# STLABTW/ST-DADK

Measured on NVIDIA B200. Metric: train_samples_per_s, higher is better.
Workload: dtype tf32

## Files before the change

st_dadk_b200/csrc/api.cu:

```cuda
#include <cstdarg>
#include <cstdio>
#include <cstring>

#include "layer.cuh"
#include "misc.cuh"
#include "sparse.cuh"
#include "predict.cuh"
#include "field.cuh"

using namespace stdadk;

static thread_local char g_err[512] = "";

static int fail(int code, const char* fmt, ...) {
    va_list ap;
    va_start(ap, fmt);
    vsnprintf(g_err, sizeof(g_err), fmt, ap);
    va_end(ap);
    return code;
}
static int check_launch(const char* what) {
    cudaError_t e = cudaGetLastError();
    if (e != cudaSuccess) return fail((int)e, "%s: %s", what, cudaGetErrorString(e));
    return 0;
// ... 16 lines not shown
    if (p.major != 10) return fail(-2, "libstdadk requires an sm_100 (B200) device, found sm_%d%d", p.major, p.minor);
    g_sm_count = p.multiProcessorCount;
    ok_dev = dev;
    return 0;
}
static int grid_for(long long work_items, int threads, int per_sm = 8) {
    long long blocks = (work_items + threads - 1) / threads;
    long long cap = (long long)(g_sm_count > 0 ? g_sm_count : 148) * per_sm;
    if (blocks > cap) blocks = cap;
    if (blocks < 1) blocks = 1;
    return (int)blocks;
}
static int pow2_cols(int n) {
    int c = 32;
    while (c < n) c <<= 1;
    return c;
}
static int tmem_cols_m64(int n_pad) { return pow2_cols((n_pad + 63) & ~63); }
template <typename K>
static int set_smem(K kernel, uint32_t bytes) {
    cudaError_t e = cudaFuncSetAttribute(kernel, cudaFuncAttributeMaxDynamicSharedMemorySize, (int)bytes);
    if (e != cudaSuccess) return fail((int)e, "cudaFuncSetAttribute(%u B smem): %s", bytes, cudaGetErrorString(e));
    return 0;
}

static BasisP to_basis(const stdadk_basis* b) {
    BasisP B{};
    if (b) {
        B.knots = reinterpret_cast<const float4*>(b->knots4);
        B.tknots = reinterpret_cast<const float2*>(b->tknots2);
        B.k_s = b->k_s;
        B.k_t = b->k_t;
        B.p_cov = b->p_cov;
        B.fn = b->basis_fn;
    }
    return B;
}
static PointsP to_points(const stdadk_points& p) {
    PointsP P{};
    P.coords = p.coords;
    P.t = p.t;
    P.xcov = p.xcov;
    P.index = reinterpret_cast<const long long*>(p.index);
    P.nx = p.grid_nx;
    P.ny = p.grid_ny;
    P.nt = p.grid_nt;
// ... 124 lines not shown
    REQUIRE(src && img && rows > 0 && cols > 0, "pack_image: bad arguments");
    REQUIRE((reinterpret_cast<uintptr_t>(img) & 127) == 0, "pack_image: image must be 128-byte aligned");
    int slabs = (int)ceil_div64(cols, SLAB_K);
    long long chunks = (long long)ceil_div64(rows, TILE_M) * slabs * (SLAB_FLOATS / 4);
    pack_image_kernel<<<grid_for(chunks, 256), 256, 0, (cudaStream_t)stream>>>(src, row_stride, col_stride, rows, cols,
                                                                                img, chunks, slabs);
    return check_launch("pack_image");
}

int stdadk_pack_images(const stdadk_pack_desc* descs, int n, void* stream) {
    if (int r = check_device()) return r;
    REQUIRE(descs && n >= 1 && n <= STDADK_MAX_PACK, "pack_images: 1..%d descriptors, got %d", STDADK_MAX_PACK, n);
    PackBatch B{};
    B.n = n;
    long long max_chunks = 0;
    for (int i = 0; i < n; ++i) {
        REQUIRE(descs[i].src && descs[i].img && descs[i].rows > 0 && descs[i].cols > 0, "pack_images: bad descriptor %d", i);
        REQUIRE((reinterpret_cast<uintptr_t>(descs[i].img) & 127) == 0, "pack_images: image %d must be 128-byte aligned", i);
        B.d[i] = descs[i];
        long long chunks = ceil_div64(descs[i].rows, TILE_M) * ceil_div64(descs[i].cols, SLAB_K) * (SLAB_FLOATS / 4);
        if (chunks > max_chunks) max_chunks = chunks;
    }
    dim3 grid(grid_for(max_chunks, 256, 2), n);
    pack_images_kernel<<<grid, 256, 0, (cudaStream_t)stream>>>(B);
    return check_launch("pack_images");
}

int stdadk_unpack_image(const float* img, int64_t rows, int64_t cols, float* dst, void* stream) {
    if (int r = check_device()) return r;
    REQUIRE(dst && img && rows > 0 && cols > 0, "unpack_image: bad arguments");
    int slabs = (int)ceil_div64(cols, SLAB_K);
    unpack_image_kernel<<<grid_for(rows * cols, 256), 256, 0, (cudaStream_t)stream>>>(img, rows, cols, dst, slabs);
    return check_launch("unpack_image");
}

static int check_layer(const stdadk_layer& l, const char* who) {
    REQUIRE(l.w_img && l.bias, "%s: weight image / bias is NULL", who);
    REQUIRE(l.n_out >= 1 && l.n_out <= MAX_N, "%s: n_out=%d outside [1,%d] (one UMMA N / LayerNorm row per thread)", who,
            l.n_out, MAX_N);
    REQUIRE(l.n_in >= 1, "%s: n_in=%d", who, l.n_in);
    REQUIRE((l.gamma == nullptr) == (l.beta == nullptr), "%s: gamma and beta must both be given or both NULL", who);
    REQUIRE(((reinterpret_cast<uintptr_t>(l.w_img) | reinterpret_cast<uintptr_t>(l.w_img_lo)) & 127) == 0,
            "%s: weight images must be 128-byte aligned", who);
    return 0;
}

constexpr uint32_t SMEM_LIMIT = 227 * 1024;
// ... 47 lines not shown
    K.dbg = g_predict_dbg;
    K.out_img = a->out_img;
    K.stats = a->stats;
    K.has_head = a->head ? 1 : 0;
    K.k_slabs = pad32(a->layer.n_in) / SLAB_K;
    K.n_pad = pad32(a->layer.n_out);
    K.thresh16 = dropout_thresh16(a->drop.p);
    K.drop_scale = a->drop.p > 0.0f ? 1.0f / (1.0f - a->drop.p) : 1.0f;
    const bool basis = a->basis != nullptr;
    int tiles = (int)ceil_div64(a->pts.n_rows, TILE_M);
    const int sms = g_sm_count > 0 ? g_sm_count : 148;
    const int cg = tiles >= 2 * sms ? 2 : 4;
    const bool half_tiles = 2 * tiles <= sms;
    if (half_tiles) tiles *= 2;
    K.tmem_cols = half_tiles ? tmem_cols_m64(K.n_pad) : pow2_cols(K.n_pad);
    const uint32_t smem = fwd_smem(K.n_pad, K.has_head ? K.head.q : 0, basis ? K.basis.k_s : 0, basis ? K.basis.k_t : 0,
                                   basis ? K.k_slabs * 8 : 0, cg);
    REQUIRE(smem <= SMEM_LIMIT, "layer_fwd: needs %u B of shared memory (> 227 KB): too many knots for the dense path",
            smem);
    K.n_tiles = tiles;
#define LAUNCH_FWD(B, TM, C)                                                                                 \
    do {                                                                                                     \
        if (int r = set_smem(layer_fwd_kernel<B, TM, C, (C == 2 ? 2 : 4)>, smem)) return r;                  \
        layer_fwd_kernel<B, TM, C, (C == 2 ? 2 : 4)><<<tiles, n_threads(C), smem, (cudaStream_t)stream>>>(K); \
    } while (0)
    if (basis) {
        if (half_tiles) LAUNCH_FWD(true, 64, 4);
        else if (cg == 2) LAUNCH_FWD(true, 128, 2);
        else LAUNCH_FWD(true, 128, 4);
    } else {
        if (half_tiles) LAUNCH_FWD(false, 64, 4);
        else if (cg == 2) LAUNCH_FWD(false, 128, 2);
        else LAUNCH_FWD(false, 128, 4);
    }
#undef LAUNCH_FWD
    return check_launch("layer_fwd");
}

extern "C" void stdadk_debug_counters(void* dev_u64x16) { g_predict_dbg = static_cast<unsigned long long*>(dev_u64x16); }

static int fill_pred_layers(const stdadk_layer* layers, int n_layers, PredLayerP* out, const char* who) {
    for (int l = 0; l < n_layers; ++l) {
        const stdadk_layer& y = layers[l];
        if (int r = check_layer(y, who)) return r;
        REQUIRE(l == 0 || y.n_in == layers[l - 1].n_out, "%s: block %d n_in=%d != previous n_out=%d", who, l, y.n_in,
                layers[l - 1].n_out);
        PredLayerP& L = out[l];
// ... 187 lines not shown
    K.d_beta = a->d_beta;
    K.d_head_w = a->d_head_w;
    K.d_head_b = a->d_head_b;
    K.has_head = a->head ? 1 : 0;
    K.k_slabs = a->x_img ? 0 : pad32(a->layer.n_in) / SLAB_K;
    K.k_slabs2 = a->head ? 0 : pad32(a->n_next) / SLAB_K;
    K.n_pad = pad32(a->layer.n_out);
    K.thresh16 = dropout_thresh16(a->drop.p);
    K.drop_scale = a->drop.p > 0.0f ? 1.0f / (1.0f - a->drop.p) : 1.0f;
    const bool basis = a->basis != nullptr && a->x_img == nullptr;
    constexpr int BCG = BWD_CG, BNS = BWD_NS;
    const uint32_t smem = bwd_smem(K.n_pad, K.has_head ? K.head.q : 0, basis ? K.basis.k_s : 0, basis ? K.basis.k_t : 0,
                                   basis ? K.k_slabs * 8 : 0);
    REQUIRE(smem <= SMEM_LIMIT, "layer_bwd: needs %u B of shared memory (> 227 KB)", smem);
    int tiles = (int)ceil_div64(a->pts.n_rows, TILE_M);
    const int sms = g_sm_count > 0 ? g_sm_count : 148;
    const bool half_tiles = a->x_img && 2 * tiles <= sms;
    if (half_tiles) tiles *= 2;
    K.tmem_cols = 2 * (half_tiles ? tmem_cols_m64(K.n_pad) : pow2_cols(K.n_pad));
    const bool ln = a->layer.gamma != nullptr, hd = a->head != nullptr;
#define LAUNCH_BWD(B, TM, LNV, HD)                                                                          \
    do {                                                                                                    \
        if (int r = set_smem(layer_bwd_kernel<B, TM, BCG, BNS, LNV, HD>, smem)) return r;                   \
        layer_bwd_kernel<B, TM, BCG, BNS, LNV, HD><<<tiles, n_threads(BCG), smem, (cudaStream_t)stream>>>(K); \
    } while (0)
    if (half_tiles) {
        if (ln && hd) LAUNCH_BWD(false, 64, true, true);
        else if (ln) LAUNCH_BWD(false, 64, true, false);
        else if (hd) LAUNCH_BWD(false, 64, false, true);
        else LAUNCH_BWD(false, 64, false, false);
    } else if (basis) {
        if (ln && hd) LAUNCH_BWD(true, 128, true, true);
        else if (ln) LAUNCH_BWD(true, 128, true, false);
        else if (hd) LAUNCH_BWD(true, 128, false, true);
        else LAUNCH_BWD(true, 128, false, false);
    } else {
        if (ln && hd) LAUNCH_BWD(false, 128, true, true);
        else if (ln) LAUNCH_BWD(false, 128, true, false);
        else if (hd) LAUNCH_BWD(false, 128, false, true);
        else LAUNCH_BWD(false, 128, false, false);
    }
#undef LAUNCH_BWD
    return check_launch("layer_bwd");
}

int stdadk_wgrad(const stdadk_wgrad_args* a, void* stream) {
    if (int r = check_device()) return r;
// ... 18 lines not shown
    K.stride_o = a->stride_o;
    K.stride_i = a->stride_i;
    K.n_in = a->n_in;
    K.n_out = a->n_out;
    K.a_slabs = pad32(a->n_in) / SLAB_K;
    K.dz_slabs = pad32(a->n_out) / SLAB_K;
    K.n_row_tiles = (int)ceil_div64(a->pts.n_rows, TILE_M);
    int n_tiles_n = (K.a_slabs + 7) / 8;
    K.nt_slabs = (K.a_slabs + n_tiles_n - 1) / n_tiles_n;
    K.tmem_cols = pow2_cols(K.nt_slabs * SLAB_K);
    int m_tiles = (K.dz_slabs + 3) / 4;
    int per = m_tiles * n_tiles_n;
    int sms = g_sm_count > 0 ? g_sm_count : 148;
    int splits = sms / per;
    if (splits < 1) splits = 1;
    if (splits > K.n_row_tiles) splits = K.n_row_tiles;
    const bool basis = a->basis != nullptr;
    uint32_t smem = wgrad_smem_bytes(basis ? K.basis.k_s : 0, basis ? K.basis.k_t : 0);
    REQUIRE(smem <= SMEM_LIMIT, "wgrad: needs %u B of shared memory (> 227 KB)", smem);
    dim3 grid(splits, m_tiles, n_tiles_n);
    constexpr int WCG = 2;
    if (basis) {
        if (int r = set_smem(wgrad_kernel<true, WCG>, smem)) return r;
        wgrad_kernel<true, WCG><<<grid, n_threads(WCG), smem, (cudaStream_t)stream>>>(K);
    } else {
        if (int r = set_smem(wgrad_kernel<false, WCG>, smem)) return r;
        wgrad_kernel<false, WCG><<<grid, n_threads(WCG), smem, (cudaStream_t)stream>>>(K);
    }
    return check_launch("wgrad");
}

static int dense_basis_check(int n_in, int n_out, int k_s, int k_t, int q_head, int training) {
    REQUIRE(n_out >= 1 && n_out <= MAX_N && k_s >= 0 && k_t >= 0 && n_in >= k_s + k_t && q_head >= 0 &&
                q_head <= STDADK_MAX_Q,
            "dense_basis_supported: bad sizes n_in=%d n_out=%d k_s=%d k_t=%d q_head=%d", n_in, n_out, k_s, k_t, q_head);
    const int n_pad = pad32(n_out), tab_chunks = pad32(n_in) / SLAB_K * 8;
    for (int cg : {4, 2}) {
        const uint32_t b = fwd_smem(n_pad, q_head, k_s, k_t, tab_chunks, cg);
        REQUIRE(b <= SMEM_LIMIT, "layer_fwd: needs %u B of shared memory (> 227 KB): too many knots for the dense path", b);
    }
    if (!training) return 0;
    const uint32_t bb = bwd_smem(n_pad, q_head, k_s, k_t, tab_chunks);
    REQUIRE(bb <= SMEM_LIMIT, "layer_bwd: needs %u B of shared memory (> 227 KB)", bb);
    const uint32_t wb = wgrad_smem_bytes(k_s, k_t);
    REQUIRE(wb <= SMEM_LIMIT, "wgrad: needs %u B of shared memory (> 227 KB)", wb);
    return 0;
}

int stdadk_dense_basis_supported(int32_t n_in, int32_t n_out, int32_t k_s, int32_t k_t, int32_t q_head, int32_t training) {
    return dense_basis_check(n_in, n_out, k_s, k_t, q_head, training) == 0 ? 1 : 0;
// ... 220 lines not shown
    K.sqnorms = a->sqnorms;
    K.step_count = a->step_count;
    K.beta1 = a->beta1;
    K.beta2 = a->beta2;
    K.eps = a->eps;
    K.ema_decay = a->ema_decay;
    K.g_zero = a->zero_grad ? const_cast<float*>(a->g) : nullptr;
    K.loss_acc = a->loss_acc;
    K.loss_sum = a->loss_sum;
    K.loss_last = a->loss_last;
    REQUIRE(((reinterpret_cast<uintptr_t>(a->p) | reinterpret_cast<uintptr_t>(a->g) | reinterpret_cast<uintptr_t>(a->m) |
              reinterpret_cast<uintptr_t>(a->v) | reinterpret_cast<uintptr_t>(a->shadow)) & 15) == 0,
            "adamw: buffers must be 16-byte aligned");
    if (a->fuse_norm) {
        REQUIRE(a->norm_ws, "adamw: fuse_norm needs norm_ws");
        K.sq_out = const_cast<float*>(a->sqnorms);
        K.norm_ws = a->norm_ws;
        K.step_rw = a->step_count;
        long long blocks = ((a->n + 3) / 4 + 255) / 256;
        if (blocks > 148) blocks = 148;
        const int sms = g_sm_count > 0 ? g_sm_count : 148;
        if (blocks > sms) blocks = sms;
        if (blocks < 1) blocks = 1;
        adamw_ema_kernel<true><<<(int)blocks, 256, 0, (cudaStream_t)stream>>>(K);
        return check_launch("adamw_ema_step (fused tail)");
    }
    step_inc_kernel<<<1, 1, 0, (cudaStream_t)stream>>>(a->step_count);
    adamw_ema_kernel<false><<<grid_for((a->n + 3) / 4, 256, 8), 256, 0, (cudaStream_t)stream>>>(K);
    return check_launch("adamw_ema_step");
}

}
```

st_dadk_b200/csrc/layer.cuh:

```cuda
#pragma once
#include "common.cuh"

namespace stdadk {

constexpr int WG_NSTAGE = 2;
constexpr int RED_STRIDE = 4 + STDADK_MAX_Q;
__host__ __device__ constexpr int n_work(int cg) { return 128 * cg; }
__host__ __device__ constexpr int n_threads(int cg) { return 128 * cg + 64; }
__device__ __forceinline__ void worker_barrier(int nw) { asm volatile("bar.sync 1, %0;" ::"r"(nw) : "memory"); }

template <int TM>
struct TileGeo {
    static_assert(TM == 128 || TM == 64, "tile height");
    static constexpr int ROWS_PER_WARP = TM / 4;
    static constexpr int WARP_COLS = TM == 128 ? 32 : 64;
    __device__ static int row(int q4, int lane) { return q4 * ROWS_PER_WARP + (TM == 128 ? lane : (lane & 15)); }
    __device__ static int chunk_off(int lane) { return TM == 128 ? 0 : (lane >> 4) * 32; }
    __device__ static int group(int cg, int lane) { return TM == 128 ? cg : 2 * cg + (lane >> 4); }
    __host__ __device__ static constexpr int groups(int cg) { return TM == 128 ? cg : 2 * cg; }
};
template <int TM>
__device__ __forceinline__ void acc_ld(uint32_t taddr, float (&v)[32]) {
    if (TM == 128) tmem_ld32(taddr, v);
    else tmem_ld16x2<32>(taddr, v);
// ... 303 lines not shown
    }
    for (; c < c_end; ++c) {
        const int f = slab * SLAB_K + 4 * c;
        const float4 v = chunk_value(chunk_kind(B, f), f);
        const uint32_t so = ((uint32_t)c ^ r7) << 4;
        st_shared_v4(rbase + so, v.x, v.y, v.z, v.w);
        if (grow) *reinterpret_cast<float4*>(grow + so) = v;
    }
}

__device__ __forceinline__ void gen_basis_slab(const BasisP& B, const float4* sk, const float2* st, int slab,
                                               float x, float y, float t, const float* xrow, uint32_t slab_saddr,
                                               uint32_t r, int c_begin = 0, int c_end = 8, float* gslab = nullptr,
                                               bool lo = false) {
#pragma unroll 1
    for (int c = c_begin; c < c_end; ++c) {
        float4 v = feature_chunk(B, sk, st, slab * SLAB_K + c * 4, x, y, t, xrow, lo);
        st_shared_v4(slab_saddr + swz_off(r, c), v.x, v.y, v.z, v.w);
        if (gslab)
            *reinterpret_cast<float4*>(reinterpret_cast<uint8_t*>(gslab) + swz_off(r, c)) = v;
    }
}

__device__ __forceinline__ void issue_slab_copies(const float* w_img, int w_slabs, int slab, int n_pad,
                                                  const float* a_tile_img, float* sA, float* sB, uint64_t* bar,
                                                  uint32_t a_bytes = SLAB_BYTES) {
    uint32_t bytes = (uint32_t)n_pad * 128u + (a_tile_img ? a_bytes : 0u);
    mbar_arrive_expect_tx(bar, bytes);
    for (int r0 = 0; r0 < n_pad; r0 += TILE_M) {
        int rows = min(TILE_M, n_pad - r0);
        const float* src = w_img + ((size_t)(r0 / TILE_M) * w_slabs + slab) * SLAB_FLOATS;
        bulk_g2s(sB + (size_t)r0 * SLAB_K, src, (uint32_t)rows * 128u, bar);
    }
    if (a_tile_img) bulk_g2s(sA, a_tile_img + (size_t)slab * SLAB_FLOATS, a_bytes, bar);
}

__device__ __forceinline__ void stage_knots_async(const BasisP& B, float4* sk, float2* st, uint64_t* bar) {
    const uint32_t ks_bytes = (uint32_t)B.k_s * 16u, kt_bytes = ((uint32_t)B.k_t >> 1) * 16u;
    mbar_arrive_expect_tx(bar, ks_bytes + kt_bytes);
    if (ks_bytes) bulk_g2s(sk, B.knots, ks_bytes, bar);
    if (kt_bytes) bulk_g2s(st, B.tknots, kt_bytes, bar);
    if (B.k_t & 1) st[B.k_t - 1] = B.tknots[B.k_t - 1];
}

__device__ __forceinline__ void issue_slab_mma(uint32_t tmem_acc, const float* sA, const float* sB, uint32_t idesc,
                                               bool first) {
    uint64_t ad = umma_desc_sw128(smem_u32(sA), 16, 1024);
    uint64_t bd = umma_desc_sw128(smem_u32(sB), 16, 1024);
#pragma unroll
    for (int k = 0; k < 4; ++k) umma_tf32(tmem_acc, ad + (uint64_t)(k * 2), bd + (uint64_t)(k * 2), idesc,
                                          (first && k == 0) ? 0u : 1u);
}

__device__ __forceinline__ bool pass_a_lo(int p) { return p == 2; }
__device__ __forceinline__ bool pass_b_lo(int p) { return p == 1; }
__device__ __forceinline__ void store_operand_chunk(float* img, float* img_lo, int tile, int slabs, int c0, uint32_t row,
                                                    const float (&v)[32]) {
// ... 376 lines not shown
    for (int i = tid; i < n_pad; i += NT) {
        bool ok = i < n_out;
        sbias[i] = ok ? P.L.bias[i] : 0.0f;
        sgam[i] = (ok && has_ln) ? P.L.gamma[i] : 1.0f;
        sbet[i] = (ok && has_ln) ? P.L.beta[i] : 0.0f;
    }
    if (P.has_head) {
        for (int i = tid; i < P.head.q * n_pad; i += NT) {
            int k = i / n_pad, c = i - k * n_pad;
            shw[i] = c < n_out ? P.head.w[(size_t)k * n_out + c] : 0.0f;
        }
        if (tid < P.head.q) shb[tid] = P.head.b[tid];
    }
    tc_fence_before();
    __syncthreads();
    tc_fence_after();
    const uint32_t tmem_base = *tmem_slot;
    FWD_T(0);

    if (warp == 4 * CG) {
        if (lane == 0) {
            const size_t a_off = (size_t)itile * P.k_slabs * SLAB_FLOATS + (size_t)irow0 * SLAB_K;
            const int n_virt = P.k_slabs * P.passes;
            for (int v = 0; v < n_virt; ++v) {
                const int s = v / P.passes, p = v - s * P.passes;
                int stage = v % NSTAGE, it = v / NSTAGE;
                if (it > 0) FWD_WAIT(7, mbar_wait(&empty[stage], (it - 1) & 1));
                const float* w_src = pass_b_lo(p) ? P.L.w_img_lo : P.L.w_img;
                const float* a_tile = BASIS ? nullptr : (pass_a_lo(p) ? P.a_img_lo : P.a_img) + a_off;
                issue_slab_copies(w_src, P.k_slabs, s, n_pad, a_tile, sA + (size_t)stage * SLAB_FLOATS,
                                  sB + stage * b_stage_floats, &full[stage], TM * 128u);
            }
        }
        __syncwarp();
    } else if (warp == 4 * CG + 1) {
        if (lane == 0) {
            const uint32_t idesc = umma_idesc_tf32((uint32_t)n_pad, 0, 0, TM);
            const int n_virt = P.k_slabs * P.passes;
            for (int s = 0; s < n_virt; ++s) {
                int stage = s % NSTAGE, it = s / NSTAGE;
                FWD_WAIT(6, mbar_wait(&full[stage], it & 1));
                tc_fence_after();
                issue_slab_mma(tmem_base, sA + (size_t)stage * SLAB_FLOATS, sB + stage * b_stage_floats, idesc,
                               s == 0);
                umma_commit(&empty[stage]);
            }
            umma_commit(accf);
        }
        __syncwarp();
    } else {
        const int q4 = warp & 3, cg = warp >> 2;
        const int row = G::row(q4, lane), grp = G::group(cg, lane);
        const long long lrow = (long long)tile * TM + row;
        const bool rvalid = tile_valid && lrow < P.pts.n_rows;
        const long long grow = P.pts.row_begin + lrow;
        if (BASIS) {
            float x = 0.f, y = 0.f, t = 0.f;
            const float* xrow = nullptr;
            if (rvalid) {
                load_point(P.pts, grow, x, y, t);
                if (P.basis.p_cov > 0 && P.pts.xcov) xrow = P.pts.xcov + sample_of(P.pts, grow) * P.basis.p_cov;
            }
            auto gen_all = [&](auto fn_tag) {
                constexpr int FN = decltype(fn_tag)::value;
                int stage = 0, it = 0;
                for (int s = 0; s < P.k_slabs; ++s) {
                    float* gslab = (P.feat_img && tile_valid)
                                       ? P.feat_img + ((size_t)itile * P.k_slabs + s) * SLAB_FLOATS + (size_t)irow0 * SLAB_K
                                       : nullptr;
                    for (int p = 0; p < P.passes; ++p) {
                        if (it > 0) {
                            if (tid == 0) FWD_WAIT(5, mbar_wait(&empty[stage], (it - 1) & 1));
                            else mbar_wait(&empty[stage], (it - 1) & 1);
// ... 100 lines not shown
    if (BASIS) build_chunk_tables(P.basis, ctab, P.k_slabs * 8, tid, NT);
    for (int i = tid; i < n_pad; i += NT) {
        bool ok = i < n_out;
        sbias[i] = ok ? P.L.bias[i] : 0.0f;
        sgam[i] = (ok && has_ln) ? P.L.gamma[i] : 1.0f;
        sbet[i] = (ok && has_ln) ? P.L.beta[i] : 0.0f;
    }
    for (int i = tid; i < (3 + q) * n_pad + STDADK_MAX_Q; i += NT) cs_bias[i] = 0.0f;
    if (HEAD) {
        for (int i = tid; i < q * n_pad; i += NT) {
            int k = i / n_pad, c = i - k * n_pad;
            shw[i] = c < n_out ? P.head.w[(size_t)k * n_out + c] : 0.0f;
        }
    }
    tc_fence_before();
    __syncthreads();
    tc_fence_after();
    const uint32_t tmem_base = *tmem_slot;

    if (warp == 4 * CG) {
        if (lane == 0) {
            const size_t a_off = (size_t)itile * P.k_slabs * SLAB_FLOATS + (size_t)irow0 * SLAB_K;
            const size_t dzn_off = (size_t)itile * P.k_slabs2 * SLAB_FLOATS + (size_t)irow0 * SLAB_K;
            for (int v = 0; v < total_slabs; ++v) {
                int stage = v % NSTAGE, it = v / NSTAGE;
                if (it > 0) mbar_wait(&empty[stage], (it - 1) & 1);
                float* a_dst = sA + (size_t)stage * SLAB_FLOATS;
                float* b_dst = sB + stage * b_stage_floats;
                if (v < virt1) {
                    const int s = v / P.passes, p = v - s * P.passes;
                    const float* a_tile = BASIS ? nullptr : (pass_a_lo(p) ? P.a_img_lo : P.a_img) + a_off;
                    issue_slab_copies(pass_b_lo(p) ? P.L.w_img_lo : P.L.w_img, P.k_slabs, s, n_pad, a_tile, a_dst, b_dst,
                                      &full[stage], TM * 128u);
                } else {
                    const int s = (v - virt1) / P.passes, p = (v - virt1) - s * P.passes;
                    issue_slab_copies(pass_b_lo(p) ? P.wt_next_img_lo : P.wt_next_img, P.k_slabs2, s, n_pad,
                                      (pass_a_lo(p) ? P.dz_next_img_lo : P.dz_next_img) + dzn_off, a_dst, b_dst, &full[stage],
                                      TM * 128u);
                }
            }
        }
        __syncwarp();
    } else if (warp == 4 * CG + 1) {
        if (lane == 0) {
            const uint32_t idesc = umma_idesc_tf32((uint32_t)n_pad, 0, 0, TM);
            for (int s = 0; s < total_slabs; ++s) {
                int stage = s % NSTAGE, it = s / NSTAGE;
                mbar_wait(&full[stage], it & 1);
                tc_fence_after();
                bool second = s >= virt1;
                issue_slab_mma(tmem_base + (second ? acc1_off : 0u), sA + (size_t)stage * SLAB_FLOATS,
                               sB + stage * b_stage_floats, idesc, s == 0 || s == virt1);
                umma_commit(&empty[stage]);
            }
            umma_commit(accf);
        }
        __syncwarp();
    } else {
        const int q4 = warp & 3, cg = warp >> 2;
        const int row = G::row(q4, lane), irow = irow0 + row, grp = G::group(cg, lane), coff = G::chunk_off(lane);
        const int c_begin = grp * (8 / NG), c_end = (grp + 1) * (8 / NG);
        const long long lrow = (long long)tile * TM + row;
        const bool rvalid = lrow < P.pts.n_rows;
// ... 8 lines not shown
            auto gen_all = [&](auto fn_tag) {
                constexpr int FN = decltype(fn_tag)::value;
                for (int v = 0; v < total_slabs; ++v) {
                    int stage = v % NSTAGE, it = v / NSTAGE;
                    if (it > 0) mbar_wait(&empty[stage], (it - 1) & 1);
                    if (v < virt1) {
                        const int s = v / P.passes, p = v - s * P.passes;
                        const uint32_t sa = smem_u32(sA + (size_t)stage * SLAB_FLOATS);
                        if (pass_a_lo(p))
                            gen_basis_slab_soa<FN, true, 2>(P.basis, ctab, s, x, y, t, xrow, sa, (uint32_t)row, c_begin,
                                                            c_end, nullptr);
                        else
                            gen_basis_slab_soa<FN, false, 2>(P.basis, ctab, s, x, y, t, xrow, sa, (uint32_t)row, c_begin,
                                                             c_end, nullptr);
                        fence_proxy_async_smem();
                    }
                    mbar_arrive_warp(&full[stage]);
                }
            };
            if (P.basis.fn == STDADK_WENDLAND) gen_all(std::integral_constant<int, STDADK_WENDLAND>{});
            else if (P.basis.fn == STDADK_TRIANGULAR) gen_all(std::integral_constant<int, STDADK_TRIANGULAR>{});
            else gen_all(std::integral_constant<int, STDADK_GAUSSIAN>{});
        }
        mbar_wait(accf, 0);
        tc_fence_after();
        const uint32_t trow = tmem_base + ((uint32_t)(q4 * 32) << 16);
        float* myred = red + ((size_t)grp * TM + row) * RED_STRIDE;
        const float* arow = (P.addend && rvalid) ? P.addend + (size_t)lrow * n_out : nullptr;
        float mean = 0.0f, rstd = 1.0f;
        if (has_ln && rvalid) {
            mean = P.stats[2 * lrow];
            rstd = P.stats[2 * lrow + 1];
        }
        float dyh[STDADK_MAX_Q];
#pragma unroll
        for (int k = 0; k < STDADK_MAX_Q; ++k)
            dyh[k] = (HEAD && rvalid && k < q) ? P.head.dyhat[lrow * q + k] : 0.0f;
        const bool drop = P.L.drop_p > 0.0f;
        const unsigned int drop_step = drop ? dropout_step(P.L) : 0u;
        const float inv_n = 1.0f / (float)n_out;
        uint32_t actbits[MAXCH];
        float Sa = 0.0f, Sb = 0.0f;
        float z[32], g[32], tmp[32];

        int ch = 0;
        for (int wc = G::WARP_COLS * cg; wc < n_pad; wc += WSTEP, ++ch) {
// ... 181 lines not shown
        if (u < units_a)
            va[j] = __ldg(reinterpret_cast<const float4*>(a_tile + (size_t)(nslab0 + (u >> 9)) * SLAB_FLOATS + hoff) + (u & 511));
    }
#pragma unroll
    for (int j = 0; j < BD; ++j) {
        const int u = tid + j * NW;
        if (u < units_d) {
            const int c = u >> 9, w = u & 511;
            const uint32_t r = (uint32_t)(w >> 3), lc = (uint32_t)(w & 7) ^ (r & 7u);
            st_shared_v4(sa + c * WG_CHUNK_BYTES + swz32_off(r, lc), vd[j].x, vd[j].y, vd[j].z, vd[j].w);
        }
    }
#pragma unroll
    for (int j = 0; j < BA; ++j) {
        const int u = tid + j * NW;
        if (u < units_a) {
            const int c = u >> 9, w = u & 511;
            const uint32_t r = (uint32_t)(w >> 3), lc = (uint32_t)(w & 7) ^ (r & 7u);
            st_shared_v4(sb + c * WG_CHUNK_BYTES + swz32_off(r, lc), va[j].x, va[j].y, va[j].z, va[j].w);
        }
    }
}

template <bool BASIS, int CG>
__global__ void __launch_bounds__(n_threads(CG), 1) wgrad_kernel(const __grid_constant__ WgradK P) {
    constexpr int NW = n_work(CG), NT = n_threads(CG);
    extern __shared__ uint8_t smem_raw[];
    uint8_t* smem = align_smem(smem_raw);
    uint8_t* stage_base = smem;
    uint64_t* full = reinterpret_cast<uint64_t*>(smem + WG_NSTAGE * WG_STAGE_BYTES);
    uint64_t* empty = full + WG_NSTAGE;
    uint64_t* accf = full + 2 * WG_NSTAGE;
    uint64_t* kbar = accf + 1;
    uint32_t* tmem_slot = reinterpret_cast<uint32_t*>(smem + WG_NSTAGE * WG_STAGE_BYTES + 64);
    float4* sk = reinterpret_cast<float4*>(smem + WG_NSTAGE * WG_STAGE_BYTES + 96);
    float2* st = reinterpret_cast<float2*>(reinterpret_cast<uint8_t*>(sk) + (size_t)(BASIS ? P.basis.k_s : 0) * 16);

    const int tid = threadIdx.x, warp = tid >> 5, lane = tid & 31;
    const int split = blockIdx.x, n_split = gridDim.x, mi = blockIdx.y, ni = blockIdx.z;
    const int m_chunks = min(4, P.dz_slabs - mi * 4);
    const int n_chunks = min(P.nt_slabs, P.a_slabs - ni * P.nt_slabs);
    const int n_mma = n_chunks * SLAB_K;
    int my_tiles = 0;
    for (int rt = split; rt < P.n_row_tiles; rt += n_split) ++my_tiles;
    const int n_iter = my_tiles * 2 * P.passes;

// ... 27 lines not shown
    if (n_iter > 0) {
        if (warp == 4 * CG + 1) {
            if (lane == 0) {
                const uint32_t idesc = umma_idesc_tf32((uint32_t)n_mma, 1, 1);
                for (int itn = 0; itn < n_iter; ++itn) {
                    int stage = itn % WG_NSTAGE, it = itn / WG_NSTAGE;
                    mbar_wait(&full[stage], it & 1);
                    tc_fence_after();
                    uint32_t sa = smem_u32(stage_base + stage * WG_STAGE_BYTES);
                    uint32_t sb = sa + WG_A_BYTES;
#pragma unroll
                    for (int k8 = 0; k8 < WG_HALF_ROWS / 8; ++k8) {
                        uint64_t ad = umma_desc_sw128_32b(sa + k8 * 1024, WG_CHUNK_BYTES, 512);
                        uint64_t bd = umma_desc_sw128_32b(sb + k8 * 1024, WG_CHUNK_BYTES, 512);
                        umma_tf32(tmem_base, ad, bd, idesc, (itn == 0 && k8 == 0) ? 0u : 1u);
                    }
                    umma_commit(&empty[stage]);
                }
                umma_commit(accf);
            }
            __syncwarp();
        } else if (warp < 4 * CG) {
            const int row64 = tid & 63, par = tid >> 6;
            int itn = 0;
            if (BASIS) mbar_wait(kbar, 0);
            for (int rt = split; rt < P.n_row_tiles; rt += n_split)
                for (int hp = 0; hp < 2 * P.passes; ++hp, ++itn) {
                    const int half = hp / P.passes, pass = hp - half * P.passes;
                    int stage = itn % WG_NSTAGE, it = itn / WG_NSTAGE;
                    float x = 0.f, y = 0.f, t = 0.f;
                    const float* xrow = nullptr;
                    if (BASIS) {
                        long long lrow = (long long)rt * TILE_M + half * WG_HALF_ROWS + row64;
                        if (lrow < P.pts.n_rows) {
                            long long grow = P.pts.row_begin + lrow;
                            load_point(P.pts, grow, x, y, t);
                            if (P.basis.p_cov > 0 && P.pts.xcov) xrow = P.pts.xcov + sample_of(P.pts, grow) * P.basis.p_cov;
                        }
                    }
                    if (it > 0) mbar_wait(&empty[stage], (it - 1) & 1);
                    uint32_t sa = smem_u32(stage_base + stage * WG_STAGE_BYTES);
                    uint32_t sb = sa + WG_A_BYTES;
                    restage_half_tiles<NW>((pass_a_lo(pass) ? P.dz_img_lo : P.dz_img) + (size_t)rt * P.dz_slabs * SLAB_FLOATS,
                                           mi * 4, m_chunks,
                                           BASIS ? nullptr
                                                 : (pass_b_lo(pass) ? P.a_img_lo : P.a_img) + (size_t)rt * P.a_slabs * SLAB_FLOATS,
                                           ni * P.nt_slabs, n_chunks, half, sa, sb, tid);
                    if (BASIS) {
                        for (int c = par; c < n_chunks; c += NW / 64) {
                            const int slab = ni * P.nt_slabs + c;
#pragma unroll 1
                            for (int c16 = 0; c16 < 8; ++c16) {
                                float4 v = feature_chunk(P.basis, sk, st, slab * SLAB_K + c16 * 4, x, y, t, xrow, pass_b_lo(pass));
                                st_shared_v4(sb + c * WG_CHUNK_BYTES + swz32_off((uint32_t)row64, (uint32_t)c16), v.x, v.y,
                                             v.z, v.w);
                            }
                        }
                    }
                    fence_proxy_async_smem();
                    mbar_arrive_warp(&full[stage]);
                }
            mbar_wait(accf, 0);
            tc_fence_after();
            const int q4 = warp & 3, cg = warp >> 2;
            const uint32_t trow = tmem_base + ((uint32_t)(q4 * 32) << 16);
            const int o = mi * TILE_M + q4 * 32 + lane;
            float v[32];
            for (int c0 = 32 * cg; c0 < n_mma; c0 += 32 * CG) {
                tmem_ld32(trow + c0, v);
                if (o < P.n_out) {
                    float* dst = P.dw + (long long)o * P.stride_o;
#pragma unroll
                    for (int i = 0; i < 32; ++i) {
                        int col = ni * P.nt_slabs * SLAB_K + c0 + i;
                        if (col < P.n_in) atomicAdd(dst + (long long)col * P.stride_i, v[i]);
                    }
                }
            }
            tc_fence_before();
        }
    }
// ... 134 lines not shown
```

st_dadk_b200/csrc/misc.cuh:

```cuda
#pragma once
#include "common.cuh"

namespace stdadk {

__global__ void pack_image_kernel(const float* __restrict__ src, long long row_stride, long long col_stride,
                                  long long rows, long long cols, float* __restrict__ img, long long n_chunks,
                                  int slabs) {
    for (long long idx = blockIdx.x * (long long)blockDim.x + threadIdx.x; idx < n_chunks;
         idx += (long long)gridDim.x * blockDim.x) {
        int chunk = (int)(idx & 7);
        int row = (int)((idx >> 3) & 127);
        long long ts = idx >> 10;
        int slab = (int)(ts % slabs);
        long long tile = ts / slabs;
        long long r = tile * TILE_M + row;
        float v[4];
#pragma unroll
        for (int e = 0; e < 4; ++e) {
            long long c = (long long)slab * SLAB_K + chunk * 4 + e;
            v[e] = (r < rows && c < cols) ? to_tf32(src[r * row_stride + c * col_stride]) : 0.0f;
        }
        float* dst = img + ts * SLAB_FLOATS;
        *reinterpret_cast<float4*>(reinterpret_cast<uint8_t*>(dst) + swz_off((uint32_t)row, (uint32_t)chunk)) =
            make_float4(v[0], v[1], v[2], v[3]);
    }
}

struct PackBatch {
    stdadk_pack_desc d[STDADK_MAX_PACK];
    int n;
};
__global__ void pack_images_kernel(PackBatch B) {
    const stdadk_pack_desc D = B.d[blockIdx.y];
    const int slabs = (int)((D.cols + SLAB_K - 1) / SLAB_K);
    const long long n_chunks = ((D.rows + TILE_M - 1) / TILE_M) * slabs * (long long)(SLAB_FLOATS / 4);
    for (long long idx = blockIdx.x * (long long)blockDim.x + threadIdx.x; idx < n_chunks;
         idx += (long long)gridDim.x * blockDim.x) {
        int chunk = (int)(idx & 7);
        int row = (int)((idx >> 3) & 127);
        long long ts = idx >> 10;
        int slab = (int)(ts % slabs);
        long long tile = ts / slabs;
        long long r = tile * TILE_M + row;
        float v[4];
#pragma unroll
        for (int e = 0; e < 4; ++e) {
            long long c = (long long)slab * SLAB_K + chunk * 4 + e;
            v[e] = (r < D.rows && c < D.cols) ? tf32_part(D.src[r * D.row_stride + c * D.col_stride], D.part != 0) : 0.0f;
        }
        float* dst = D.img + ts * SLAB_FLOATS;
        *reinterpret_cast<float4*>(reinterpret_cast<uint8_t*>(dst) + swz_off((uint32_t)row, (uint32_t)chunk)) =
            make_float4(v[0], v[1], v[2], v[3]);
    }
}

// ... 301 lines not shown
    const float* g;
    float* m;
    float* v;
    float* shadow;
    long long n;
    GroupsP G;
    const float* hyper;
    const float* sqnorms;
    const int* step_count;
    float beta1, beta2, eps, ema_decay;
    float* g_zero;
    float* loss_acc;
    float* loss_sum;
    float* loss_last;
    float* sq_out;
    float* norm_ws;
    int* step_rw;
};
template <bool FUSED>
__global__ void __launch_bounds__(256) adamw_ema_kernel(AdamK A) {
    __shared__ float s_sq[8];
    int step;
    if (FUSED) {
        step = *A.step_count + 1;
        float acc[8];
#pragma unroll
        for (int k = 0; k < 8; ++k) acc[k] = 0.0f;
        if (A.sqnorms) {
            const long long n4q = A.n >> 2;
            const float4* gq = reinterpret_cast<const float4*>(A.g);
            for (long long i = blockIdx.x * (long long)blockDim.x + threadIdx.x; i < n4q; i += (long long)gridDim.x * blockDim.x) {
                const float4 v = __ldg(gq + i);
                const long long e = i << 2;
                const float vv[4] = {v.x, v.y, v.z, v.w};
#pragma unroll
                for (int j = 0; j < 4; ++j) {
                    const int gi = group_of(A.G, e + j);
#pragma unroll
                    for (int k = 0; k < 8; ++k)
                        if (k == gi) acc[k] = fmaf(vv[j], vv[j], acc[k]);
                }
            }
            if (blockIdx.x == 0 && threadIdx.x < (A.n & 3)) {
                const long long i = (n4q << 2) + threadIdx.x;
                const float v = A.g[i];
                const int gi = group_of(A.G, i);
// ... 118 lines not shown
```

st_dadk_b200/csrc/ptx.cuh:

```cuda
#pragma once
#include <cuda_runtime.h>
#include <stdint.h>

namespace stdadk {

__device__ __forceinline__ uint32_t smem_u32(const void* p) {
    return static_cast<uint32_t>(__cvta_generic_to_shared(p));
}

__device__ __forceinline__ void mbar_init(uint64_t* bar, uint32_t count) {
    asm volatile("mbarrier.init.shared::cta.b64 [%0], %1;" ::"r"(smem_u32(bar)), "r"(count) : "memory");
}
__device__ __forceinline__ void mbar_fence_init() {
    asm volatile("fence.mbarrier_init.release.cluster;" ::: "memory");
}
__device__ __forceinline__ void mbar_arrive(uint64_t* bar) {
    asm volatile("mbarrier.arrive.shared::cta.b64 _, [%0];" ::"r"(smem_u32(bar)) : "memory");
}
__device__ __forceinline__ void mbar_arrive_warp(uint64_t* bar) {
    __syncwarp();
    if ((threadIdx.x & 31u) == 0u) mbar_arrive(bar);
}
__device__ __forceinline__ void mbar_arrive_expect_tx(uint64_t* bar, uint32_t bytes) {
    asm volatile("mbarrier.arrive.expect_tx.shared::cta.b64 _, [%0], %1;" ::"r"(smem_u32(bar)), "r"(bytes)
                 : "memory");
}
__device__ __forceinline__ bool mbar_try_wait(uint64_t* bar, uint32_t parity, uint32_t hint_ns = 20000u) {
    uint32_t ok;
    asm volatile(
        "{\n\t.reg .pred p;\n\t"
        "mbarrier.try_wait.parity.shared::cta.b64 p, [%1], %2, %3;\n\t"
        "selp.b32 %0, 1, 0, p;\n\t}"
        : "=r"(ok)
        : "r"(smem_u32(bar)), "r"(parity), "r"(hint_ns)
        : "memory");
    return ok != 0;
}
__device__ __forceinline__ void mbar_wait(uint64_t* bar, uint32_t parity) {
    if (mbar_try_wait(bar, parity)) return;
    long long t0 = clock64();
    while (!mbar_try_wait(bar, parity)) {
        if (clock64() - t0 > 4000000000LL) __trap();
    }
}

__device__ __forceinline__ void fence_proxy_async_smem() {
    asm volatile("fence.proxy.async.shared::cta;" ::: "memory");
}
__device__ __forceinline__ void tc_fence_before() {
    asm volatile("tcgen05.fence::before_thread_sync;" ::: "memory");
}
__device__ __forceinline__ void tc_fence_after() {
    asm volatile("tcgen05.fence::after_thread_sync;" ::: "memory");
}

__device__ __forceinline__ void bulk_g2s(void* smem_dst, const void* gsrc, uint32_t bytes, uint64_t* bar) {
    asm volatile("cp.async.bulk.shared::cluster.global.mbarrier::complete_tx::bytes [%0], [%1], %2, [%3];" ::"r"(
                     smem_u32(smem_dst)),
                 "l"(gsrc), "r"(bytes), "r"(smem_u32(bar))
                 : "memory");
}

__device__ __forceinline__ void tmem_alloc(uint32_t* smem_dst, uint32_t ncols) {
    asm volatile("tcgen05.alloc.cta_group::1.sync.aligned.shared::cta.b32 [%0], %1;" ::"r"(smem_u32(smem_dst)),
                 "r"(ncols)
                 : "memory");
    asm volatile("tcgen05.relinquish_alloc_permit.cta_group::1.sync.aligned;" ::: "memory");
// ... 148 lines not shown
```

st_dadk_b200/executor.py:

```python
from __future__ import annotations

import ctypes as C
from dataclasses import dataclass
from typing import Dict, List, Optional, Sequence, Tuple

import torch

from . import _lib as L
from . import ops


@dataclass
class NetSpec:
    centers: torch.Tensor
    bandwidths: Optional[torch.Tensor]
    log_bandwidths: Optional[torch.Tensor]
    t_centers: torch.Tensor
    t_bandwidths: torch.Tensor
    weights: List[torch.Tensor]
    biases: List[torch.Tensor]
    gammas: List[Optional[torch.Tensor]]
    betas: List[Optional[torch.Tensor]]
    head_w: torch.Tensor
    head_b: torch.Tensor
# ... 517 lines not shown
            a.drop = drop
            if ws.x is not None:
                a.x_img = ws.x[l].data_ptr()
            if ws.stats[l] is not None:
                a.stats = ws.stats[l].data_ptr()
                a.d_gamma = g["gammas"][l].data_ptr()
                a.d_beta = g["betas"][l].data_ptr()
            if l == nh - 1:
                a.head = C.pointer(head)
                a.d_head_w = g["head_w"].data_ptr()
                a.d_head_b = g["head_b"].data_ptr()
            else:
                a.dz_next_img = ws.dz[l + 1].data_ptr()
                a.wt_next_img = self.wt_img[l + 1].data_ptr()
                a.n_next = s.weights[l + 1].shape[0]
                if self.x3:
                    a.dz_next_img_lo = ws.dz_lo[l + 1].data_ptr()
                    a.wt_next_img_lo = self.wt_img_lo[l + 1].data_ptr()
            a.dz_img = ws.dz[l].data_ptr()
            if self.x3:
                a.dz_img_lo = ws.dz_lo[l].data_ptr()
            a.d_bias = g["biases"][l].data_ptr()
            ops.layer_bwd(a)
            side.wait_stream(main)
            with torch.cuda.stream(side):
                self._wgrad_block(l, pts, ws, basis, g)
        main.wait_stream(side)
        if s.learnable_basis and not self.sparse:
            a = L.KnotGradArgs()
            a.basis = C.pointer(basis)
            a.pts = pts
            a.dz_img = ws.dz[0].data_ptr()
            a.w1s_img = self.w1s_img.data_ptr()
            if self.x3:
                a.dz_img_lo = ws.dz_lo[0].data_ptr()
                a.w1s_img_lo = self.w1s_img_lo.data_ptr()
            a.n_out = s.weights[0].shape[0]
            a.d_centers = g["centers"].data_ptr()
            a.d_log_bw = g["log_bandwidths"].data_ptr()
            ops.knot_grad(a)
        return g
```

Before: 24.20 million.

## Add programmatic dependent launch to overlap kernel prologues with predecessors

Launches the forward, backward, wgrad, pack and fused AdamW kernels with programmatic stream serialization, enabled only when the grid fits in one wave. Inside the kernels, weight-slab copies and basis-feature generation that don't depend on the previous kernel are issued before griddepcontrol.wait, and activation slabs follow it. This hides launch latency and prologue work. The last layer's wgrad now runs on the main stream instead of the side stream so it can chain with PDL. The risk is ordering bugs if anything read before the wait depends on the predecessor, and less overlap for layer 0's wgrad.

```diff
diff --git a/st_dadk_b200/csrc/api.cu b/st_dadk_b200/csrc/api.cu
--- a/st_dadk_b200/csrc/api.cu
+++ b/st_dadk_b200/csrc/api.cu
@@ -62,6 +62,23 @@
     cudaError_t e = cudaFuncSetAttribute(kernel, cudaFuncAttributeMaxDynamicSharedMemorySize, (int)bytes);
     if (e != cudaSuccess) return fail((int)e, "cudaFuncSetAttribute(%u B smem): %s", bytes, cudaGetErrorString(e));
     return 0;
+}
+
+template <typename... KArgs, typename... Args>
+static void launch_chained(void (*kernel)(KArgs...), dim3 grid, int threads, uint32_t smem, void* stream,
+                           Args&&... args) {
+    const long long ctas = (long long)grid.x * grid.y * grid.z;
+    cudaLaunchAttribute attr[1];
+    attr[0].id = cudaLaunchAttributeProgrammaticStreamSerialization;
+    attr[0].val.programmaticStreamSerializationAllowed = ctas <= (g_sm_count > 0 ? g_sm_count : 148) ? 1 : 0;
+    cudaLaunchConfig_t cfg{};
+    cfg.gridDim = grid;
+    cfg.blockDim = dim3(threads);
+    cfg.dynamicSmemBytes = smem;
+    cfg.stream = (cudaStream_t)stream;
+    cfg.attrs = attr;
+    cfg.numAttrs = 1;
+    (void)cudaLaunchKernelEx(&cfg, kernel, std::forward<Args>(args)...);
 }
 
 static BasisP to_basis(const stdadk_basis* b) {
@@ -232,7 +249,7 @@
         if (chunks > max_chunks) max_chunks = chunks;
     }
     dim3 grid(grid_for(max_chunks, 256, 2), n);
-    pack_images_kernel<<<grid, 256, 0, (cudaStream_t)stream>>>(B);
+    launch_chained(pack_images_kernel, grid, 256, 0, stream, B);
     return check_launch("pack_images");
 }
 
@@ -326,7 +343,7 @@
 #define LAUNCH_FWD(B, TM, C)                                                                                 \
     do {                                                                                                     \
         if (int r = set_smem(layer_fwd_kernel<B, TM, C, (C == 2 ? 2 : 4)>, smem)) return r;                  \
-        layer_fwd_kernel<B, TM, C, (C == 2 ? 2 : 4)><<<tiles, n_threads(C), smem, (cudaStream_t)stream>>>(K); \
+        launch_chained(layer_fwd_kernel<B, TM, C, (C == 2 ? 2 : 4)>, dim3(tiles), n_threads(C), smem, stream, K); \
     } while (0)
     if (basis) {
         if (half_tiles) LAUNCH_FWD(true, 64, 4);
@@ -560,7 +577,7 @@
 #define LAUNCH_BWD(B, TM, LNV, HD)                                                                          \
     do {                                                                                                    \
         if (int r = set_smem(layer_bwd_kernel<B, TM, BCG, BNS, LNV, HD>, smem)) return r;                   \
-        layer_bwd_kernel<B, TM, BCG, BNS, LNV, HD><<<tiles, n_threads(BCG), smem, (cudaStream_t)stream>>>(K); \
+        launch_chained(layer_bwd_kernel<B, TM, BCG, BNS, LNV, HD>, dim3(tiles), n_threads(BCG), smem, stream, K); \
     } while (0)
     if (half_tiles) {
         if (ln && hd) LAUNCH_BWD(false, 64, true, true);
@@ -625,10 +642,10 @@
     constexpr int WCG = 2;
     if (basis) {
         if (int r = set_smem(wgrad_kernel<true, WCG>, smem)) return r;
-        wgrad_kernel<true, WCG><<<grid, n_threads(WCG), smem, (cudaStream_t)stream>>>(K);
+        launch_chained(wgrad_kernel<true, WCG>, grid, n_threads(WCG), smem, stream, K);
     } else {
         if (int r = set_smem(wgrad_kernel<false, WCG>, smem)) return r;
-        wgrad_kernel<false, WCG><<<grid, n_threads(WCG), smem, (cudaStream_t)stream>>>(K);
+        launch_chained(wgrad_kernel<false, WCG>, grid, n_threads(WCG), smem, stream, K);
     }
     return check_launch("wgrad");
 }
@@ -895,7 +912,7 @@
         const int sms = g_sm_count > 0 ? g_sm_count : 148;
         if (blocks > sms) blocks = sms;
         if (blocks < 1) blocks = 1;
-        adamw_ema_kernel<true><<<(int)blocks, 256, 0, (cudaStream_t)stream>>>(K);
+        launch_chained(adamw_ema_kernel<true>, dim3((unsigned)blocks), 256, 0, stream, K);
         return check_launch("adamw_ema_step (fused tail)");
     }
     step_inc_kernel<<<1, 1, 0, (cudaStream_t)stream>>>(a->step_count);
diff --git a/st_dadk_b200/csrc/layer.cuh b/st_dadk_b200/csrc/layer.cuh
--- a/st_dadk_b200/csrc/layer.cuh
+++ b/st_dadk_b200/csrc/layer.cuh
@@ -349,9 +349,13 @@
     }
 }
 
+__device__ __forceinline__ void issue_a_slab(int slab, const float* a_tile_img, float* sA, uint64_t* bar,
+                                             uint32_t a_bytes) {
+    bulk_g2s(sA, a_tile_img + (size_t)slab * SLAB_FLOATS, a_bytes, bar);
+}
 __device__ __forceinline__ void issue_slab_copies(const float* w_img, int w_slabs, int slab, int n_pad,
                                                   const float* a_tile_img, float* sA, float* sB, uint64_t* bar,
-                                                  uint32_t a_bytes = SLAB_BYTES) {
+                                                  uint32_t a_bytes = SLAB_BYTES, bool a_later = false) {
     uint32_t bytes = (uint32_t)n_pad * 128u + (a_tile_img ? a_bytes : 0u);
     mbar_arrive_expect_tx(bar, bytes);
     for (int r0 = 0; r0 < n_pad; r0 += TILE_M) {
@@ -359,7 +363,7 @@
         const float* src = w_img + ((size_t)(r0 / TILE_M) * w_slabs + slab) * SLAB_FLOATS;
         bulk_g2s(sB + (size_t)r0 * SLAB_K, src, (uint32_t)rows * 128u, bar);
     }
-    if (a_tile_img) bulk_g2s(sA, a_tile_img + (size_t)slab * SLAB_FLOATS, a_bytes, bar);
+    if (a_tile_img && !a_later) issue_a_slab(slab, a_tile_img, sA, bar, a_bytes);
 }
 
 __device__ __forceinline__ void stage_knots_async(const BasisP& B, float4* sk, float2* st, uint64_t* bar) {
@@ -782,7 +786,21 @@
         if (lane == 0) {
             const size_t a_off = (size_t)itile * P.k_slabs * SLAB_FLOATS + (size_t)irow0 * SLAB_K;
             const int n_virt = P.k_slabs * P.passes;
-            for (int v = 0; v < n_virt; ++v) {
+            const int n_pre = BASIS ? 0 : min(n_virt, NSTAGE);
+            for (int v = 0; v < n_pre; ++v) {
+                const int s = v / P.passes, p = v - s * P.passes;
+                issue_slab_copies(pass_b_lo(p) ? P.L.w_img_lo : P.L.w_img, P.k_slabs, s, n_pad,
+                                  (pass_a_lo(p) ? P.a_img_lo : P.a_img) + a_off, sA + (size_t)v * SLAB_FLOATS,
+                                  sB + v * b_stage_floats, &full[v], TM * 128u, true);
+            }
+            pdl_wait();
+            pdl_launch_dependents();
+            for (int v = 0; v < n_pre; ++v) {
+                const int s = v / P.passes, p = v - s * P.passes;
+                issue_a_slab(s, (pass_a_lo(p) ? P.a_img_lo : P.a_img) + a_off, sA + (size_t)v * SLAB_FLOATS, &full[v],
+                             TM * 128u);
+            }
+            for (int v = n_pre; v < n_virt; ++v) {
                 const int s = v / P.passes, p = v - s * P.passes;
                 int stage = v % NSTAGE, it = v / NSTAGE;
                 if (it > 0) FWD_WAIT(7, mbar_wait(&empty[stage], (it - 1) & 1));
@@ -809,6 +827,7 @@
         }
         __syncwarp();
     } else {
+        pdl_wait();
         const int q4 = warp & 3, cg = warp >> 2;
         const int row = G::row(q4, lane), grp = G::group(cg, lane);
         const long long lrow = (long long)tile * TM + row;
@@ -955,7 +974,18 @@
         if (lane == 0) {
             const size_t a_off = (size_t)itile * P.k_slabs * SLAB_FLOATS + (size_t)irow0 * SLAB_K;
             const size_t dzn_off = (size_t)itile * P.k_slabs2 * SLAB_FLOATS + (size_t)irow0 * SLAB_K;
+            const int n_pre = min(total_slabs, NSTAGE);
+            auto wait_then_dz_next = [&]() {
+                pdl_wait();
+                pdl_launch_dependents();
+                for (int v = virt1; v < n_pre; ++v) {
+                    const int s = (v - virt1) / P.passes, p = (v - virt1) - s * P.passes;
+                    issue_a_slab(s, (pass_a_lo(p) ? P.dz_next_img_lo : P.dz_next_img) + dzn_off,
+                                 sA + (size_t)v * SLAB_FLOATS, &full[v], TM * 128u);
+                }
+            };
             for (int v = 0; v < total_slabs; ++v) {
+                if (v == n_pre) wait_then_dz_next();
                 int stage = v % NSTAGE, it = v / NSTAGE;
                 if (it > 0) mbar_wait(&empty[stage], (it - 1) & 1);
                 float* a_dst = sA + (size_t)stage * SLAB_FLOATS;
@@ -969,9 +999,10 @@
                     const int s = (v - virt1) / P.passes, p = (v - virt1) - s * P.passes;
                     issue_slab_copies(pass_b_lo(p) ? P.wt_next_img_lo : P.wt_next_img, P.k_slabs2, s, n_pad,
                                       (pass_a_lo(p) ? P.dz_next_img_lo : P.dz_next_img) + dzn_off, a_dst, b_dst, &full[stage],
-                                      TM * 128u);
+                                      TM * 128u, v < n_pre);
                 }
             }
+            if (total_slabs == n_pre) wait_then_dz_next();
         }
         __syncwarp();
     } else if (warp == 4 * CG + 1) {
@@ -1026,6 +1057,7 @@
             else if (P.basis.fn == STDADK_TRIANGULAR) gen_all(std::integral_constant<int, STDADK_TRIANGULAR>{});
             else gen_all(std::integral_constant<int, STDADK_GAUSSIAN>{});
         }
+        pdl_wait();
         mbar_wait(accf, 0);
         tc_fence_after();
         const uint32_t trow = tmem_base + ((uint32_t)(q4 * 32) << 16);
@@ -1253,6 +1285,28 @@
     }
 }
 
+template <int NW>
+__device__ __noinline__ void wgrad_gen_basis_half(const WgradK& P, const float4* sk, const float2* st, int rt, int half,
+                                                  int pass, uint32_t sb, int row64, int par, int n_chunks) {
+    float x = 0.f, y = 0.f, t = 0.f;
+    const float* xrow = nullptr;
+    long long lrow = (long long)rt * TILE_M + half * WG_HALF_ROWS + row64;
+    if (lrow < P.pts.n_rows) {
+        long long grow = P.pts.row_begin + lrow;
+        load_point(P.pts, grow, x, y, t);
+        if (P.basis.p_cov > 0 && P.pts.xcov) xrow = P.pts.xcov + sample_of(P.pts, grow) * P.basis.p_cov;
+    }
+    const int ni = blockIdx.z;
+    for (int c = par; c < n_chunks; c += NW / 64) {
+        const int slab = ni * P.nt_slabs + c;
+#pragma unroll 1
+        for (int c16 = 0; c16 < 8; ++c16) {
+            float4 v = feature_chunk(P.basis, sk, st, slab * SLAB_K + c16 * 4, x, y, t, xrow, pass_b_lo(pass));
+            st_shared_v4(sb + c * WG_CHUNK_BYTES + swz32_off((uint32_t)row64, (uint32_t)c16), v.x, v.y, v.z, v.w);
+        }
+    }
+}
+
 template <bool BASIS, int CG>
 __global__ void __launch_bounds__(n_threads(CG), 1) wgrad_kernel(const __grid_constant__ WgradK P) {
     constexpr int NW = n_work(CG), NT = n_threads(CG);
@@ -1326,22 +1380,25 @@
             __syncwarp();
         } else if (warp < 4 * CG) {
             const int row64 = tid & 63, par = tid >> 6;
+            auto gen_basis = [&](int rt, int half, int pass, int stage) {
+                wgrad_gen_basis_half<NW>(P, sk, st, rt, half, pass, smem_u32(stage_base + stage * WG_STAGE_BYTES) + WG_A_BYTES,
+                                         row64, par, n_chunks);
+            };
+            const int n_pre = BASIS ? min(n_iter, WG_NSTAGE) : 0;
             int itn = 0;
-            if (BASIS) mbar_wait(kbar, 0);
+            if (BASIS) {
+                mbar_wait(kbar, 0);
+                for (int rt = split; rt < P.n_row_tiles && itn < n_pre; rt += n_split)
+                    for (int hp = 0; hp < 2 * P.passes && itn < n_pre; ++hp, ++itn)
+                        gen_basis(rt, hp / P.passes, hp % P.passes, itn);
+            }
+            pdl_wait();
+            pdl_launch_dependents();
+            itn = 0;
             for (int rt = split; rt < P.n_row_tiles; rt += n_split)
                 for (int hp = 0; hp < 2 * P.passes; ++hp, ++itn) {
                     const int half = hp / P.passes, pass = hp - half * P.passes;
                     int stage = itn % WG_NSTAGE, it = itn / WG_NSTAGE;
-                    float x = 0.f, y = 0.f, t = 0.f;
-                    const float* xrow = nullptr;
-                    if (BASIS) {
-                        long long lrow = (long long)rt * TILE_M + half * WG_HALF_ROWS + row64;
-                        if (lrow < P.pts.n_rows) {
-                            long long grow = P.pts.row_begin + lrow;
-                            load_point(P.pts, grow, x, y, t);
-                            if (P.basis.p_cov > 0 && P.pts.xcov) xrow = P.pts.xcov + sample_of(P.pts, grow) * P.basis.p_cov;
-                        }
-                    }
                     if (it > 0) mbar_wait(&empty[stage], (it - 1) & 1);
                     uint32_t sa = smem_u32(stage_base + stage * WG_STAGE_BYTES);
                     uint32_t sb = sa + WG_A_BYTES;
@@ -1350,17 +1407,7 @@
                                            BASIS ? nullptr
                                                  : (pass_b_lo(pass) ? P.a_img_lo : P.a_img) + (size_t)rt * P.a_slabs * SLAB_FLOATS,
                                            ni * P.nt_slabs, n_chunks, half, sa, sb, tid);
-                    if (BASIS) {
-                        for (int c = par; c < n_chunks; c += NW / 64) {
-                            const int slab = ni * P.nt_slabs + c;
-#pragma unroll 1
-                            for (int c16 = 0; c16 < 8; ++c16) {
-                                float4 v = feature_chunk(P.basis, sk, st, slab * SLAB_K + c16 * 4, x, y, t, xrow, pass_b_lo(pass));
-                                st_shared_v4(sb + c * WG_CHUNK_BYTES + swz32_off((uint32_t)row64, (uint32_t)c16), v.x, v.y,
-                                             v.z, v.w);
-                            }
-                        }
-                    }
+                    if (BASIS && itn >= n_pre) gen_basis(rt, half, pass, stage);
                     fence_proxy_async_smem();
                     mbar_arrive_warp(&full[stage]);
                 }
diff --git a/st_dadk_b200/csrc/misc.cuh b/st_dadk_b200/csrc/misc.cuh
--- a/st_dadk_b200/csrc/misc.cuh
+++ b/st_dadk_b200/csrc/misc.cuh
@@ -31,6 +31,8 @@
     int n;
 };
 __global__ void pack_images_kernel(PackBatch B) {
+    pdl_wait();
+    pdl_launch_dependents();
     const stdadk_pack_desc D = B.d[blockIdx.y];
     const int slabs = (int)((D.cols + SLAB_K - 1) / SLAB_K);
     const long long n_chunks = ((D.rows + TILE_M - 1) / TILE_M) * slabs * (long long)(SLAB_FLOATS / 4);
@@ -378,6 +380,7 @@
     __shared__ float s_sq[8];
     int step;
     if (FUSED) {
+        pdl_wait();
         step = *A.step_count + 1;
         float acc[8];
 #pragma unroll
diff --git a/st_dadk_b200/csrc/ptx.cuh b/st_dadk_b200/csrc/ptx.cuh
--- a/st_dadk_b200/csrc/ptx.cuh
+++ b/st_dadk_b200/csrc/ptx.cuh
@@ -43,6 +43,9 @@
         if (clock64() - t0 > 4000000000LL) __trap();
     }
 }
+
+__device__ __forceinline__ void pdl_wait() { asm volatile("griddepcontrol.wait;" ::: "memory"); }
+__device__ __forceinline__ void pdl_launch_dependents() { asm volatile("griddepcontrol.launch_dependents;" ::: "memory"); }
 
 __device__ __forceinline__ void fence_proxy_async_smem() {
     asm volatile("fence.proxy.async.shared::cta;" ::: "memory");
diff --git a/st_dadk_b200/executor.py b/st_dadk_b200/executor.py
--- a/st_dadk_b200/executor.py
+++ b/st_dadk_b200/executor.py
@@ -563,9 +563,12 @@
                 a.dz_img_lo = ws.dz_lo[l].data_ptr()
             a.d_bias = g["biases"][l].data_ptr()
             ops.layer_bwd(a)
-            side.wait_stream(main)
-            with torch.cuda.stream(side):
+            if l == 0:
                 self._wgrad_block(l, pts, ws, basis, g)
+            else:
+                side.wait_stream(main)
+                with torch.cuda.stream(side):
+                    self._wgrad_block(l, pts, ws, basis, g)
         main.wait_stream(side)
         if s.learnable_basis and not self.sparse:
             a = L.KnotGradArgs()
```

Measured after the change: 27.95 million, median of 6. 1.15x the previous value.
